# NVIDIA/k8s-operator-libs

Hardware: AMD Instinct MI355X
Metric: 8-node rolling-upgrade wall-clock (lower is better)
Workload: dtype fp32; 1 GPU; model=amdgpu-driver-rolling-upgrade, nodes_per_cluster=8, maxParallelUpgrades=2, maxUnavailable=50%, drain=True, podDeletion=True, gpu_pods_per_node=2, gpu_validation=True, converging_reconcile=True, mode=inplace, global_batch=8, parallelism=dp1 (one independent simulated 8-node cluster per rank)

## Files before the change

k8s_operator_libs_amd/core/restclient.py:

```python

from __future__ import annotations

import collections
import http.client as _http_client
import json
import os
from typing import Any, Dict, Optional

import httpx

from ..native import load_wire as _load_wire
from . import meta
from .client import Client
from .errors import (
    AlreadyExistsError,
    ApiError,
    BadRequestError,
    ConflictError,
    NotFoundError,
)

SA_DIR = "/var/run/secrets/kubernetes.io/serviceaccount"

_KIND_INFO = {
    ("v1", "Node"): ("nodes", False),
    ("v1", "Pod"): ("pods", True),
    ("v1", "Event"): ("events", True),
    ("v1", "Namespace"): ("namespaces", False),
    ("apps/v1", "DaemonSet"): ("daemonsets", True),
    ("apps/v1", "ControllerRevision"): ("controllerrevisions", True),
    ("apiextensions.k8s.io/v1", "CustomResourceDefinition"): (
        "customresourcedefinitions", False),
    ("maintenance.amd.com/v1alpha1", "NodeMaintenance"): ("nodemaintenances", True),
    ("coordination.k8s.io/v1", "Lease"): ("leases", True),
}


def _lower_plural(kind: str) -> str:
    k = kind.lower()
    if k.endswith(("ss", "x", "z", "ch", "sh")):
        return k + "es"
    if k.endswith("s"):
        return k
    if k.endswith("y") and len(k) > 1 and k[-2] not in "aeiou":
        return k[:-1] + "ies"
    return k + "s"


class RestClient(Client):
    def __init__(
        self,
        base_url: str,
        token: Optional[str] = None,
        verify: Any = True,
        timeout: float = 30.0,
        extra_kinds: Optional[Dict[tuple, tuple]] = None,
        retries: int = 3,
    ) -> None:
        self.base_url = base_url.rstrip("/")
        headers = {"Content-Type": "application/json"}
        if token:
            headers["Authorization"] = f"Bearer {token}"
        self._headers = dict(headers)
        self._timeout = timeout
        self._http = httpx.Client(
            base_url=self.base_url, headers=headers, verify=verify, timeout=timeout
        )
        self._fast_netloc = None
        self._wire = None
        if self.base_url.startswith("http://"):
            import urllib.parse

            parsed = urllib.parse.urlsplit(self.base_url)
            self._fast_netloc = (parsed.hostname, parsed.port or 80)
            self._fast_local = __import__("threading").local()
            self._wire = _load_wire()
            self._wire_heads: Dict[tuple, bytes] = {}
        self._kinds = dict(_KIND_INFO)
        if extra_kinds:
            self._kinds.update(extra_kinds)
        self._retries = retries


    def _wire_head(self, headers=None) -> bytes:
        key = tuple(sorted(headers.items())) if headers else ()
        head = self._wire_heads.get(key)
        if head is None:
            host, port = self._fast_netloc
            if ":" in host:
                host = f"[{host}]"
            hdrs = {"Host": host if port == 80 else f"{host}:{port}",
                    "Accept-Encoding": "identity"}
            hdrs.update(self._headers)
            if headers:
                hdrs.update(headers)
            head = "".join(f"{k}: {v}\r\n" for k, v in hdrs.items()).encode(
                "latin-1")
            self._wire_heads[key] = head
        return head

    def _wire_connect(self):
        import socket

        sock = socket.create_connection(self._fast_netloc,
                                        timeout=self._timeout)
        sock.setsockopt(socket.IPPROTO_TCP, socket.TCP_NODELAY, 1)
        return sock

    def _wire_request(self, method: str, path: str, params=None, content=None,
                      headers=None):
        import urllib.parse

        if params:
            path = f"{path}?{urllib.parse.urlencode(params)}"
        head = self._wire_head(headers)
        sock = getattr(self._fast_local, "sock", None)
        for attempt in (0, 1):
            try:
                if sock is None:
                    sock = self._wire_connect()
                    self._fast_local.sock = sock
                status, data, reusable = self._wire.exchange(
                    sock.fileno(), method, path, head, content, self._timeout)
            except ValueError as exc:
                self._wire_drop(sock)
                raise _http_client.HTTPException(str(exc)) from exc
            except (ConnectionError, OSError):
                self._wire_drop(sock)
                sock = None
                if attempt:
                    raise
            except BaseException:
                self._wire_drop(sock)
                raise
            else:
                if not reusable:
                    self._wire_drop(sock)
                return _FastResponse(status, data)
        raise AssertionError("unreachable")

    def _wire_drop(self, sock) -> None:
        if sock is not None:
            try:
                sock.close()
            except Exception:
                pass
        self._fast_local.sock = None

    def _fast_request(self, method: str, path: str, params=None, content=None,
                      headers=None):
        if self._wire is not None:
            return self._wire_request(method, path, params=params,
                                      content=content, headers=headers)
        import http.client
        import urllib.parse

        if params:
            path = f"{path}?{urllib.parse.urlencode(params)}"
        conn = getattr(self._fast_local, "conn", None)
        hdrs = dict(self._headers)
        if headers:
            hdrs.update(headers)
        body = content if content is not None else None
        for attempt in (0, 1):
            if conn is None:
                conn = http.client.HTTPConnection(
                    *self._fast_netloc, timeout=self._timeout
                )
                self._fast_local.conn = conn
            try:
                conn.request(method, path, body=body, headers=hdrs)
                resp = conn.getresponse()
                data = resp.read()
                return _FastResponse(resp.status, data)
            except (http.client.HTTPException, ConnectionError, OSError):
                try:
                    conn.close()
                except Exception:
                    pass
                conn = None
                self._fast_local.conn = None
                if attempt:
                    raise
        raise AssertionError("unreachable")

    def _request(self, method: str, path: str, **kw) -> httpx.Response:
        import time as _time

        attempt = 0
        while True:
            try:
                if self._fast_netloc is not None:
                    resp = self._fast_request(method, path, **kw)
                else:
                    resp = self._http.request(method, path, **kw)
            except (httpx.ConnectError, httpx.ReadError, httpx.RemoteProtocolError,
                    httpx.ConnectTimeout, httpx.ReadTimeout,
                    _http_client.HTTPException,
                    ConnectionError, OSError) as exc:
                if attempt >= self._retries:
                    err = ApiError(f"connection to apiserver failed: {exc}")
                    err.code = 503
                    raise err from exc
            else:
                if resp.status_code not in (429, 500, 502, 503, 504) or \
                        attempt >= self._retries:
                    return resp
            attempt += 1
            _time.sleep(min(0.05 * (2 ** attempt), 1.0))

    @classmethod
    def from_environment(cls) -> "RestClient":
        token_path = os.path.join(SA_DIR, "token")
        if os.path.exists(token_path):
            with open(token_path) as fh:
                token = fh.read().strip()
            host = os.environ.get("KUBERNETES_SERVICE_HOST", "kubernetes.default.svc")
            port = os.environ.get("KUBERNETES_SERVICE_PORT", "443")
            ca = os.path.join(SA_DIR, "ca.crt")
            return cls(f"https://{host}:{port}", token=token,
                       verify=ca if os.path.exists(ca) else True)
# ... 136 lines not shown
        return resp.json()

    def update(self, obj):
        api_version, kind = meta.api_version(obj), meta.kind(obj)
        path = self._object_path(api_version, kind, meta.name(obj), meta.namespace(obj))
        resp = self._request("PUT", path, content=json.dumps(obj))
        self._raise_for(resp)
        return resp.json()

    def patch(self, api_version, kind, name, patch, namespace=""):
        path = self._object_path(api_version, kind, name, namespace)
        resp = self._request(
            "PATCH", path, content=json.dumps(patch),
            headers={"Content-Type": "application/merge-patch+json"},
        )
        self._raise_for(resp)
        return resp.json()

    def delete(self, api_version, kind, name, namespace="", grace_period_seconds=None):
        kw = {}
        if grace_period_seconds is not None:
            kw["content"] = json.dumps({
                "apiVersion": "v1", "kind": "DeleteOptions",
                "gracePeriodSeconds": int(grace_period_seconds),
            })
        resp = self._request(
            "DELETE", self._object_path(api_version, kind, name, namespace), **kw
        )
        self._raise_for(resp)

    def patch_status(self, api_version, kind, name, status, namespace=""):
        path = self._object_path(api_version, kind, name, namespace) + "/status"
        resp = self._request(
            "PATCH", path, content=json.dumps({"status": status}),
            headers={"Content-Type": "application/merge-patch+json"},
        )
        self._raise_for(resp)
        return resp.json()

    def evict_pod(self, name, namespace):
        path = self._object_path("v1", "Pod", name, namespace) + "/eviction"
        body = {
            "apiVersion": "policy/v1",
            "kind": "Eviction",
            "metadata": {"name": name, "namespace": namespace},
        }
        resp = self._request("POST", path, content=json.dumps(body))
        self._raise_for(resp)

    def watch(self, api_version: str, kind: str, namespace=None,
              resource_version=None, label_selector="", field_selector="",
              send_initial_events=False):
        return _HttpWatch(self, api_version, kind, namespace=namespace,
                          resource_version=resource_version,
                          label_selector=label_selector,
                          field_selector=field_selector,
                          send_initial_events=send_initial_events)


    def discover_resource(self, api_version: str, plural: str) -> bool:
        prefix = f"/api/{api_version}" if "/" not in api_version else f"/apis/{api_version}"
        resp = self._request("GET", prefix)
        if resp.status_code != 200:
            return False
        for res in resp.json().get("resources", []):
            if res.get("name") == plural:
                return True
        return False

    def register_kind(self, api_version: str, kind: str, plural: str, namespaced: bool) -> None:
        self._kinds[(api_version, kind)] = (plural, namespaced)

    def close(self) -> None:
        self._http.close()
        if self._fast_netloc is not None:
            conn = getattr(self._fast_local, "conn", None)
            if conn is not None:
                try:
                    conn.close()
                except Exception:
                    pass
                self._fast_local.conn = None
            self._wire_drop(getattr(self._fast_local, "sock", None))


class _FastResponse:

    __slots__ = ("status_code", "_data")

    def __init__(self, status_code: int, data: bytes) -> None:
        self.status_code = status_code
        self._data = data

    def json(self):
        return json.loads(self._data)

    @property
    def text(self) -> str:
        return self._data.decode(errors="replace")


class _HttpWatch:

    USE_LINE_PUMP = True

    def __init__(self, client: RestClient, api_version: str, kind: str,
                 namespace=None, resource_version=None,
                 label_selector="", field_selector="",
                 send_initial_events=False) -> None:
        import queue
        import threading

        self._queue: "queue.Queue" = queue.Queue()
        self._stop = threading.Event()
        self._connected = threading.Event()
        path = client._collection_path(api_version, kind, namespace or "")
        params = {"watch": "true", "allowWatchBookmarks": "true"}
        if resource_version is not None:
            params["resourceVersion"] = str(resource_version)
        if label_selector:
            params["labelSelector"] = label_selector
        if field_selector:
            params["fieldSelector"] = field_selector
        if send_initial_events:
            params["sendInitialEvents"] = "true"
            params["resourceVersionMatch"] = "NotOlderThan"
        self._error: Optional[BaseException] = None

        def reader():
            try:
                with client._http.stream(
                    "GET", path, params=params, timeout=None,
                ) as resp:
                    self._resp = resp
                    if resp.status_code == 410:
                        from .errors import GoneError

                        self._error = GoneError("watch resume point expired")
                        return
                    if resp.status_code >= 400:
                        err = ApiError(f"watch rejected: HTTP {resp.status_code}")
                        err.code = resp.status_code
                        self._error = err
                        return
                    self._connected.set()
                    for line in resp.iter_lines():
                        if self._stop.is_set():
                            break
                        line = line.strip()
                        if not line:
                            continue
                        try:
                            event = json.loads(line)
                        except ValueError:
                            continue
                        self._queue.put((event.get("type"), event.get("object")))
            except Exception as exc:
                if not self._stop.is_set():
                    import logging as _logging

                    _logging.getLogger(__name__).warning(
                        "watch stream ended: %s", exc
                    )
            finally:
                self._connected.set()

# ... 237 lines not shown
```

k8s_operator_libs_amd/native/build.py:

```python

from __future__ import annotations

import os
import subprocess
import sysconfig

PKG_DIR = os.path.dirname(os.path.abspath(__file__))
SOURCE = os.path.join(PKG_DIR, "gpu_validator.hip")
OUTPUT = os.path.join(PKG_DIR, "_gpu_validator.so")
JSONOPS_SOURCE = os.path.join(PKG_DIR, "jsonops.cpp")
JSONOPS_OUTPUT = os.path.join(PKG_DIR, "_jsonops.so")
WIRE_SOURCES = (
    os.path.join(PKG_DIR, "wire.cpp"),
    os.path.join(PKG_DIR, "wire_core.hpp"),
    os.path.join(PKG_DIR, "wire_stream.hpp"),
)
WIRE_OUTPUT = os.path.join(PKG_DIR, "_wire.so")

HIPCC = os.environ.get("HIPCC", "/opt/rocm/bin/hipcc")
CXX = os.environ.get("CXX", "g++")


def validator_sources() -> list:
    wire = {os.path.basename(p) for p in WIRE_SOURCES}
    return [SOURCE] + sorted(
        os.path.join(PKG_DIR, name) for name in os.listdir(PKG_DIR)
        if name.endswith(".hpp") and name not in wire)


def is_built() -> bool:
    return os.path.exists(OUTPUT) and all(
        os.path.getmtime(OUTPUT) >= os.path.getmtime(src)
        for src in validator_sources())


def build_jsonops(force: bool = False, verbose: bool = False) -> str:
    if (
        not force
        and os.path.exists(JSONOPS_OUTPUT)
        and os.path.getmtime(JSONOPS_OUTPUT) >= os.path.getmtime(JSONOPS_SOURCE)
    ):
        return JSONOPS_OUTPUT
    cmd = [
        CXX, "-O3", "-std=c++17", "-fPIC", "-shared",
        f"-I{sysconfig.get_paths()['include']}",
        JSONOPS_SOURCE, "-o", JSONOPS_OUTPUT,
    ]
    if verbose:
        print(" ".join(cmd))
    subprocess.run(cmd, check=True, capture_output=not verbose)
    return JSONOPS_OUTPUT


def build_wire(force: bool = False, verbose: bool = False) -> str:
    if (
        not force
        and os.path.exists(WIRE_OUTPUT)
        and all(os.path.getmtime(WIRE_OUTPUT) >= os.path.getmtime(src)
                for src in WIRE_SOURCES)
    ):
        return WIRE_OUTPUT
    cmd = [
        CXX, "-O3", "-std=c++17", "-fPIC", "-shared", "-pthread",
        f"-I{sysconfig.get_paths()['include']}",
        WIRE_SOURCES[0], "-o", WIRE_OUTPUT,
    ]
    if verbose:
        print(" ".join(cmd))
    subprocess.run(cmd, check=True, capture_output=not verbose)
    return WIRE_OUTPUT


def build(force: bool = False, verbose: bool = False) -> str:
    build_jsonops(force=force, verbose=verbose)
    build_wire(force=force, verbose=verbose)
    if is_built() and not force:
        return OUTPUT
    import pybind11

    cmd = [
        HIPCC,
        "--offload-arch=gfx950",
        "-O3",
        "-std=c++17",
        "-fPIC",
        "-shared",
        f"-I{sysconfig.get_paths()['include']}",
        f"-I{pybind11.get_include()}",
        SOURCE,
        "-o",
        OUTPUT,
    ]
    if verbose:
        print(" ".join(cmd))
    subprocess.run(cmd, check=True, capture_output=not verbose)
    return OUTPUT

# ... 5 lines not shown
```

k8s_operator_libs_amd/native/wire.cpp:

```cpp

#define PY_SSIZE_T_CLEAN
#include <Python.h>

#include <atomic>
#include <cerrno>
#include <chrono>
#include <memory>
#include <mutex>
#include <new>
#include <string>
#include <system_error>
#include <thread>
#include <vector>

#include <fcntl.h>
#include <poll.h>
#include <sys/socket.h>
#include <sys/types.h>
#include <unistd.h>

#include "wire_core.hpp"
#include "wire_stream.hpp"

namespace {

constexpr size_t kRecvBuf = 64 * 1024;

using Clock = std::chrono::steady_clock;

struct Deadline {
  bool infinite;
  Clock::time_point at;

  explicit Deadline(double timeout_s) : infinite(timeout_s < 0) {
    if (!infinite)
      at = Clock::now() + std::chrono::duration_cast<Clock::duration>(
                              std::chrono::duration<double>(timeout_s));
  }

  int remaining_ms() const {
    if (infinite) return -1;
    auto left = std::chrono::duration_cast<std::chrono::microseconds>(
                    at - Clock::now()).count();
    if (left <= 0) return 0;
    long long ms = (left + 999) / 1000;
    return ms > 0x7fffffff ? 0x7fffffff : int(ms);
  }
};

bool parse_timeout(PyObject* obj, double* out) {
  if (obj == nullptr || obj == Py_None) {
    *out = -1.0;
    return true;
  }
  double v = PyFloat_AsDouble(obj);
  if (v == -1.0 && PyErr_Occurred()) return false;
  *out = v < 0 ? 0.0 : v;
  return true;
}

enum IoResult { kIoOk = 0, kIoTimeout = 1, kIoError = 2, kIoSignal = 3 };

IoResult wait_fd(int fd, short events, const Deadline& dl) {
  for (;;) {
    int ms = dl.remaining_ms();
    struct pollfd p = {fd, events, 0};
    int rc, err;
    Py_BEGIN_ALLOW_THREADS
    rc = poll(&p, 1, ms);
    err = errno;
    Py_END_ALLOW_THREADS
    if (rc > 0) return kIoOk;
    if (rc == 0) {
      if (ms != 0 && dl.remaining_ms() != 0) continue;
      return kIoTimeout;
    }
    if (err == EINTR) {
      if (PyErr_CheckSignals() < 0) return kIoSignal;
      continue;
    }
    errno = err;
    PyErr_SetFromErrno(PyExc_OSError);
    return kIoError;
  }
}

IoResult recv_some(int fd, char* buf, size_t cap, const Deadline& dl,
                   size_t* got) {
  for (;;) {
    int ms = dl.remaining_ms();
    struct pollfd p = {fd, POLLIN, 0};
    int rc, err;
    ssize_t n = -1;
    Py_BEGIN_ALLOW_THREADS
    rc = poll(&p, 1, ms);
    err = errno;
    if (rc > 0) {
      n = recv(fd, buf, cap, MSG_DONTWAIT);
      err = errno;
    }
    Py_END_ALLOW_THREADS
    if (rc == 0) {
      if (ms != 0 && dl.remaining_ms() != 0) continue;
      return kIoTimeout;
    }
    if (n >= 0) {
      *got = size_t(n);
      return kIoOk;
    }
    if (rc > 0 && (err == EAGAIN || err == EWOULDBLOCK)) continue;
    if (err == EINTR) {
      if (PyErr_CheckSignals() < 0) return kIoSignal;
      continue;
    }
    errno = err;
    PyErr_SetFromErrno(PyExc_OSError);
    return kIoError;
  }
}

IoResult send_all(int fd, const char* buf, size_t len, const Deadline& dl) {
  size_t off = 0;
  while (off < len) {
    ssize_t n;
    int err;
    Py_BEGIN_ALLOW_THREADS
    n = send(fd, buf + off, len - off, MSG_NOSIGNAL | MSG_DONTWAIT);
    err = errno;
    Py_END_ALLOW_THREADS
    if (n >= 0) {
      off += size_t(n);
      continue;
    }
    if (err == EAGAIN || err == EWOULDBLOCK) {
      IoResult w = wait_fd(fd, POLLOUT, dl);
      if (w != kIoOk) return w;
      continue;
    }
    if (err == EINTR) {
      if (PyErr_CheckSignals() < 0) return kIoSignal;
      continue;
    }
    errno = err;
    PyErr_SetFromErrno(PyExc_OSError);
    return kIoError;
  }
  return kIoOk;
}

PyObject* raise_wire_error(int st) {
  PyErr_SetString(PyExc_ValueError, wire::status_message(st));
  return nullptr;
}

PyObject* raise_timeout() {
  PyErr_SetString(PyExc_TimeoutError, "timed out");
  return nullptr;
}

bool status_has_no_body(int status) {
  return status == 204 || status == 304;
}

bool as_buffer(PyObject* obj, const char** p, Py_ssize_t* n, bool* present) {
  *present = true;
  if (obj == Py_None) {
    *p = "";
    *n = 0;
    *present = false;
    return true;
  }
  if (PyBytes_Check(obj)) {
    *p = PyBytes_AS_STRING(obj);
    *n = PyBytes_GET_SIZE(obj);
    return true;
  }
  if (PyUnicode_Check(obj)) {
    *p = PyUnicode_AsUTF8AndSize(obj, n);
    return *p != nullptr;
  }
  PyErr_SetString(PyExc_TypeError, "body must be bytes, str or None");
  return false;
}


PyObject* py_exchange(PyObject* , PyObject* args) {
  int fd;
  const char *method, *path, *head;
  Py_ssize_t method_len, path_len, head_len;
  PyObject *body_obj, *timeout_obj = Py_None;
  if (!PyArg_ParseTuple(args, "is#s#y#O|O", &fd, &method, &method_len, &path,
                        &path_len, &head, &head_len, &body_obj, &timeout_obj))
    return nullptr;
  const char* body;
  Py_ssize_t body_len;
  bool has_body;
  if (!as_buffer(body_obj, &body, &body_len, &has_body)) return nullptr;
  double timeout_s;
  if (!parse_timeout(timeout_obj, &timeout_s)) return nullptr;
  Deadline dl(timeout_s);

  std::string method_s(method, size_t(method_len));
  bool is_head = method_s == "HEAD";
  bool wants_length = has_body || method_s == "POST" || method_s == "PUT" ||
                      method_s == "PATCH";

  std::string req;
  req.reserve(size_t(method_len + path_len + head_len + body_len) + 64);
  req.append(method_s).append(" ").append(path, size_t(path_len));
  req.append(" HTTP/1.1\r\n").append(head, size_t(head_len));
  if (wants_length)
    req.append("Content-Length: ").append(std::to_string(body_len)).append("\r\n");
  req.append("\r\n").append(body, size_t(body_len));

  IoResult io = send_all(fd, req.data(), req.size(), dl);
  if (io == kIoTimeout) return raise_timeout();
  if (io != kIoOk) return nullptr;

  wire::HeadParser head_parser(wire::HeadParser::kResponse);
  wire::ChunkedDecoder chunked;
  std::string out;
  enum { kHead, kLength, kChunked, kUntilClose, kComplete } phase = kHead;
  size_t remaining = 0;
  bool reusable = true;
  bool got_any = false;
  char buf[kRecvBuf];

  while (phase != kComplete) {
    size_t got = 0;
    io = recv_some(fd, buf, sizeof buf, dl, &got);
    if (io == kIoTimeout) return raise_timeout();
    if (io != kIoOk) return nullptr;
    if (got == 0) {
      if (phase == kUntilClose) {
        phase = kComplete;
        break;
      }
      PyErr_SetString(got_any ? PyExc_ConnectionError
                              : PyExc_ConnectionResetError,
                      got_any ? "peer closed the connection mid-response"
                              : "peer closed the connection without a response");
      return nullptr;
    }
    got_any = true;
    const char* p = buf;
    size_t n = got;
    while (n > 0 && phase != kComplete) {
      size_t used = 0;
      if (phase == kHead) {
        int st = head_parser.feed(p, n, &used);
        if (st < 0) return raise_wire_error(st);
        if (st == wire::kDone) {
          int code = head_parser.status;
          if (code >= 100 && code < 200 && code != 101) {
            head_parser.reset();
          } else {
            if (!head_parser.keep_alive()) reusable = false;
            if (is_head || status_has_no_body(code)) {
              phase = kComplete;
            } else if (head_parser.chunked) {
              phase = kChunked;
            } else if (head_parser.has_content_length) {
              remaining = head_parser.content_length;
              if (remaining == 0) {
                phase = kComplete;
              } else {
                phase = kLength;
                out.reserve(remaining < (size_t(1) << 26) ? remaining
                                                          : (size_t(1) << 26));
              }
            } else {
              phase = kUntilClose;
              reusable = false;
            }
          }
        }
      } else if (phase == kLength) {
        used = n < remaining ? n : remaining;
        out.append(p, used);
        remaining -= used;
        if (remaining == 0) phase = kComplete;
      } else if (phase == kChunked) {
        int st = chunked.feed(p, n, &used, &out);
        if (st < 0) return raise_wire_error(st);
        if (st == wire::kDone) phase = kComplete;
      } else {
        used = n;
        out.append(p, used);
      }
      p += used;
      n -= used;
    }
    if (n > 0) reusable = false;
  }

  PyObject* body_bytes =
      PyBytes_FromStringAndSize(out.data(), Py_ssize_t(out.size()));
  if (!body_bytes) return nullptr;
  PyObject* res = Py_BuildValue("(iNO)", head_parser.status, body_bytes,
                                reusable ? Py_True : Py_False);
  return res;
}


PyObject* py_parse_request_head(PyObject* , PyObject* arg) {
  Py_buffer view;
  if (PyObject_GetBuffer(arg, &view, PyBUF_SIMPLE) < 0) return nullptr;
  wire::HeadParser hp(wire::HeadParser::kRequest);
  size_t used = 0;
  int st = hp.feed(static_cast<const char*>(view.buf), size_t(view.len), &used);
  PyBuffer_Release(&view);
  if (st < 0) return raise_wire_error(st);
  if (st == wire::kNeedMore) Py_RETURN_NONE;
  PyObject* length;
  if (hp.has_content_length) {
    length = PyLong_FromSize_t(hp.content_length);
    if (!length) return nullptr;
  } else {
    length = Py_None;
    Py_INCREF(length);
  }
  return Py_BuildValue("(s#s#iNOOn)", hp.method.data(),
                       Py_ssize_t(hp.method.size()), hp.target.data(),
                       Py_ssize_t(hp.target.size()), hp.version_minor, length,
                       hp.chunked ? Py_True : Py_False,
                       hp.keep_alive() ? Py_True : Py_False,
                       Py_ssize_t(used));
}


struct LineReaderObject {
  PyObject_HEAD
  int fd;
  bool busy;
  wire::LineFramer* framer;
  std::string* buf;
};

void linereader_dealloc(LineReaderObject* self) {
  delete self->framer;
  delete self->buf;
  Py_TYPE(self)->tp_free(reinterpret_cast<PyObject*>(self));
}

int linereader_init(LineReaderObject* self, PyObject* args, PyObject* ) {
  int fd;
  if (!PyArg_ParseTuple(args, "i", &fd)) return -1;
  if (self->framer != nullptr) {
    PyErr_SetString(PyExc_RuntimeError, "LineReader is already initialised");
    return -1;
  }
  self->fd = fd;
  self->busy = false;
  try {
    self->framer = new wire::LineFramer();
    self->buf = new std::string(kRecvBuf, '\0');
  } catch (const std::bad_alloc&) {
    PyErr_NoMemory();
    return -1;
  }
  return 0;
}

IoResult linereader_fill(LineReaderObject* self, const Deadline& dl) {
  size_t got = 0;
  self->busy = true;
  IoResult io = recv_some(self->fd, &(*self->buf)[0], self->buf->size(), dl,
                          &got);
  self->busy = false;
  if (io != kIoOk) return io;
  if (got == 0) {
    self->framer->peer_closed();
    return kIoOk;
  }
  try {
    int st = self->framer->consume(self->buf->data(), got);
    if (st < 0) {
      raise_wire_error(st);
      return kIoError;
    }
  } catch (const std::bad_alloc&) {
    PyErr_NoMemory();
    return kIoError;
// ... 568 lines not shown
        std::make_shared<Stream>(fd, size_t(max_backlog)));
  } catch (const std::bad_alloc&) {
    PyErr_NoMemory();
    return -1;
  }
  self->closed = false;
  return 0;
}

PyObject* streamwriter_write(StreamWriterObject* self, PyObject* arg) {
  if (self->stream == nullptr) {
    PyErr_SetString(PyExc_RuntimeError, "StreamWriter is not initialised");
    return nullptr;
  }
  Py_buffer view;
  if (PyObject_GetBuffer(arg, &view, PyBUF_SIMPLE) < 0) return nullptr;
  bool ok = false;
  if (!self->closed) {
    const std::shared_ptr<Stream>& s = *self->stream;
    Stream* raw = s.get();
    try {
      auto st = raw->buf.write(
          static_cast<const char*>(view.buf), size_t(view.len),
          [raw](const char* p, size_t n) { return raw->send_some(p, n); });
      if (st == wire::StreamBuffer::kQueued && !Flusher::instance().attach(s)) {
        raw->buf.kill();
        st = wire::StreamBuffer::kDead;
      }
      if (st == wire::StreamBuffer::kDead) raw->on_dead();
      ok = st != wire::StreamBuffer::kDead;
    } catch (const std::bad_alloc&) {
      raw->buf.kill();
      raw->on_dead();
    }
  }
  PyBuffer_Release(&view);
  return PyBool_FromLong(ok);
}

PyObject* streamwriter_close(StreamWriterObject* self, PyObject*) {
  if (self->stream != nullptr && !self->closed) {
    self->closed = true;
    Flusher::instance().detach(*self->stream);
  }
  Py_RETURN_NONE;
}

PyObject* streamwriter_get_dead(StreamWriterObject* self, void*) {
  if (self->stream == nullptr) Py_RETURN_TRUE;
  return PyBool_FromLong(self->closed || (*self->stream)->buf.dead());
}

PyObject* streamwriter_get_pending(StreamWriterObject* self, void*) {
  if (self->stream == nullptr) return PyLong_FromLong(0);
  return PyLong_FromSize_t((*self->stream)->buf.pending());
}

PyMethodDef streamwriter_methods[] = {
    {"write", reinterpret_cast<PyCFunction>(streamwriter_write), METH_O,
     "write(data) -> bool.  Thread-safe, never blocks, never raises for a "
     "broken stream.  With nothing queued the bytes are sent on the calling "
     "thread; what the socket does not take waits in the backlog, which one "
     "native thread per process drains on POLLOUT.  Each call's bytes reach "
     "the peer contiguously.  False once the writer is dead or closed."},
    {"close", reinterpret_cast<PyCFunction>(streamwriter_close), METH_NOARGS,
     "close().  Detach from the flusher thread; on return nothing native "
     "uses the fd any more.  Unsent backlog is dropped."},
    {nullptr, nullptr, 0, nullptr},
};

PyGetSetDef streamwriter_getset[] = {
    {"dead", reinterpret_cast<getter>(streamwriter_get_dead), nullptr,
     "True after a send error, a backlog past max_backlog (the socket is "
     "then shut down, not closed) or close()", nullptr},
    {"pending", reinterpret_cast<getter>(streamwriter_get_pending), nullptr,
     "bytes waiting in the backlog", nullptr},
    {nullptr, nullptr, nullptr, nullptr, nullptr},
};

PyTypeObject StreamWriterType = {
    PyVarObject_HEAD_INIT(nullptr, 0)
    "_wire.StreamWriter",
    sizeof(StreamWriterObject),
};


PyObject* py_exchange_guarded(PyObject* self, PyObject* args) {
  try {
    return py_exchange(self, args);
  } catch (const std::bad_alloc&) {
    return PyErr_NoMemory();
  }
}

PyObject* py_parse_request_head_guarded(PyObject* self, PyObject* arg) {
  try {
    return py_parse_request_head(self, arg);
  } catch (const std::bad_alloc&) {
    return PyErr_NoMemory();
  }
}

PyMethodDef wire_methods[] = {
    {"exchange", py_exchange_guarded, METH_VARARGS,
     "exchange(fd, method, path, header_bytes, body, timeout=None) -> "
     "(status, body_bytes, reusable).  One HTTP/1.1 request/response on a "
     "connected socket: the request goes out in a single send; the response "
     "is read with Content-Length, chunked or read-to-EOF framing.  "
     "reusable is False when the connection must not carry another request."},
    {"parse_request_head", py_parse_request_head_guarded, METH_O,
     "parse_request_head(data) -> None | (method, target, minor_version, "
     "content_length | None, chunked, keep_alive, head_size).  None while "
     "the head is incomplete; ValueError when it is malformed."},
    {nullptr, nullptr, 0, nullptr},
};

struct PyModuleDef wire_module = {
    PyModuleDef_HEAD_INIT, "_wire",
    "Native HTTP/1.1 framing for the REST client and the watch reader", -1,
    wire_methods,
};

}

PyMODINIT_FUNC PyInit__wire(void) {
  LineReaderType.tp_flags = Py_TPFLAGS_DEFAULT;
  LineReaderType.tp_doc =
      "LineReader(fd): newline-delimited reader over a streaming HTTP "
      "response on a socket the caller owns (never closed here).";
  LineReaderType.tp_new = PyType_GenericNew;
  LineReaderType.tp_init = reinterpret_cast<initproc>(linereader_init);
  LineReaderType.tp_dealloc = reinterpret_cast<destructor>(linereader_dealloc);
  LineReaderType.tp_methods = linereader_methods;
  LineReaderType.tp_getset = linereader_getset;
  if (PyType_Ready(&LineReaderType) < 0) return nullptr;
  StreamWriterType.tp_flags = Py_TPFLAGS_DEFAULT;
  StreamWriterType.tp_doc =
      "StreamWriter(fd, max_backlog=64 MiB): non-blocking, thread-safe line "
      "writer over a socket the caller owns (never closed here).  The "
      "default cap holds the replay that opens a watch, which is written in "
      "one go, and equals the 64 MiB cap on a single line; a reader further "
      "behind than that is cut off and re-watches.";
  StreamWriterType.tp_new = PyType_GenericNew;
  StreamWriterType.tp_init = reinterpret_cast<initproc>(streamwriter_init);
  StreamWriterType.tp_dealloc =
      reinterpret_cast<destructor>(streamwriter_dealloc);
  StreamWriterType.tp_methods = streamwriter_methods;
  StreamWriterType.tp_getset = streamwriter_getset;
  if (PyType_Ready(&StreamWriterType) < 0) return nullptr;
  LinePumpType.tp_flags = Py_TPFLAGS_DEFAULT;
  LinePumpType.tp_doc =
      "LinePump(fd | LineReader): one native thread reads the response head "
      "and then lines from a socket the caller owns, without ever taking "
      "the GIL; consumers wait() for the line count to move and drain().  "
      "Given a LineReader, the thread reads through it and the reader is "
      "the pump's from then on.  To end it: shut the socket down, stop(), "
      "and only then close the socket.";
  LinePumpType.tp_new = PyType_GenericNew;
  LinePumpType.tp_init = reinterpret_cast<initproc>(linepump_init);
  LinePumpType.tp_dealloc = reinterpret_cast<destructor>(linepump_dealloc);
  LinePumpType.tp_methods = linepump_methods;
  LinePumpType.tp_getset = linepump_getset;
  if (PyType_Ready(&LinePumpType) < 0) return nullptr;
  PyObject* m = PyModule_Create(&wire_module);
  if (!m) return nullptr;
  Py_INCREF(&LinePumpType);
  if (PyModule_AddObject(m, "LinePump",
                         reinterpret_cast<PyObject*>(&LinePumpType)) < 0) {
    Py_DECREF(&LinePumpType);
    Py_DECREF(m);
    return nullptr;
  }
  Py_INCREF(&StreamWriterType);
  if (PyModule_AddObject(m, "StreamWriter",
                         reinterpret_cast<PyObject*>(&StreamWriterType)) < 0) {
    Py_DECREF(&StreamWriterType);
    Py_DECREF(m);
    return nullptr;
  }
  Py_INCREF(&LineReaderType);
  if (PyModule_AddObject(m, "LineReader",
                         reinterpret_cast<PyObject*>(&LineReaderType)) < 0) {
    Py_DECREF(&LineReaderType);
    Py_DECREF(m);
    return nullptr;
  }
  return m;
}
```

k8s_operator_libs_amd/native/wire_core.hpp:

```cpp

#pragma once

#include <cstddef>
#include <cstdint>
#include <cstring>
#include <string>

namespace wire {

enum Status : int {
  kNeedMore = 0,
  kDone = 1,
  kErrHeadTooLarge = -1,
  kErrBadHead = -2,
  kErrBadLength = -3,
  kErrBadChunk = -4,
  kErrLineTooLong = -5,
};

inline const char* status_message(int st) {
  switch (st) {
    case kNeedMore: return "need more input";
    case kDone: return "done";
    case kErrHeadTooLarge: return "HTTP head larger than 64 KiB";
// ... 239 lines not shown
            state_ = kSizeLF;
          } else if (c == ';' || detail::is_ows(c)) {
            state_ = kExt;
          } else {
            return fail(consumed, i);
          }
          if (++meta_len_ > kMaxHead) return fail(consumed, i);
          break;
        }
        case kExt:
          if (c == '\r') state_ = kSizeLF;
          else if (c == '\n') return fail(consumed, i);
          if (++meta_len_ > kMaxHead) return fail(consumed, i);
          break;
        case kSizeLF:
          if (c != '\n') return fail(consumed, i);
          meta_len_ = 0;
          if (remaining_ == 0) {
            state_ = kTrailer;
            trailer_line_len_ = 0;
          } else {
            state_ = kData;
          }
          break;
        case kDataCR:
          if (c != '\r') return fail(consumed, i);
          state_ = kDataLF;
          break;
        case kDataLF:
          if (c != '\n') return fail(consumed, i);
          state_ = kSizeFirst;
          break;
        case kTrailer:
          if (c == '\r') state_ = kTrailerLF;
          else if (c == '\n') return fail(consumed, i);
          else ++trailer_line_len_;
          if (++meta_len_ > kMaxHead) return fail(consumed, i);
          break;
        case kTrailerLF:
          if (c != '\n') return fail(consumed, i);
          if (trailer_line_len_ == 0) {
            state_ = kEnd;
          } else {
            state_ = kTrailer;
            trailer_line_len_ = 0;
          }
          break;
        default:
          return fail(consumed, i);
      }
    }
    *consumed = i;
    return state_ == kEnd ? kDone : kNeedMore;
  }

  bool done() const { return state_ == kEnd; }

 private:
  enum State {
    kSizeFirst, kSize, kExt, kSizeLF, kData, kDataCR, kDataLF,
    kTrailer, kTrailerLF, kEnd, kFailed,
  };

  static int hex(char c) {
    if (c >= '0' && c <= '9') return c - '0';
    if (c >= 'a' && c <= 'f') return c - 'a' + 10;
    if (c >= 'A' && c <= 'F') return c - 'A' + 10;
    return -1;
  }

  int fail(size_t* consumed, size_t i) {
    state_ = kFailed;
    *consumed = i;
    return kErrBadChunk;
  }

  State state_;
  size_t remaining_;
  size_t meta_len_;
  size_t trailer_line_len_;
};


class LineSplitter {
 public:
  explicit LineSplitter(size_t max_line = kMaxLine)
      : max_line_(max_line), pos_(0), scan_(0) {}

  void feed(const char* data, size_t n) {
    if (pos_ > 0 && pos_ == buf_.size()) {
      buf_.clear();
      pos_ = scan_ = 0;
    }
    buf_.append(data, n);
  }

  int next(std::string* out) {
    for (;;) {
      const char* base = buf_.data();
      const char* lf = scan_ < buf_.size()
          ? static_cast<const char*>(
                std::memchr(base + scan_, '\n', buf_.size() - scan_))
          : nullptr;
      if (!lf) {
        scan_ = buf_.size();
        if (buf_.size() - pos_ > max_line_) return kErrLineTooLong;
        if (pos_ > 0) {
          buf_.erase(0, pos_);
          scan_ -= pos_;
          pos_ = 0;
        }
        return kNeedMore;
      }
      size_t end = size_t(lf - base);
      size_t start = pos_;
      pos_ = scan_ = end + 1;
      if (end - start > max_line_) return kErrLineTooLong;
      if (strip(base, start, end, out)) return kDone;
    }
  }

  int flush(std::string* out) {
    size_t start = pos_, end = buf_.size();
    pos_ = scan_ = end;
    if (end - start > max_line_) return kErrLineTooLong;
    return strip(buf_.data(), start, end, out) ? kDone : kNeedMore;
  }

  size_t pending() const { return buf_.size() - pos_; }

 private:
  static bool is_space(char c) {
    return c == ' ' || c == '\t' || c == '\r' || c == '\n' || c == '\f' ||
           c == '\v';
  }

  static bool strip(const char* base, size_t start, size_t end,
                    std::string* out) {
    while (start < end && is_space(base[start])) ++start;
    while (end > start && is_space(base[end - 1])) --end;
    if (start == end) return false;
    out->assign(base + start, end - start);
    return true;
  }

  size_t max_line_;
  std::string buf_;
  size_t pos_;
  size_t scan_;
};

}
```

Before: 25.12 ms.

## Share keep-alive connections across threads via a native connection pool

Adds a native C++ Pool that keeps idle keep-alive sockets to the API server and lends them to any thread. Before, each thread kept its own socket. Threads in the concurrent drain, pod and node workers can now reuse warm connections instead of dialing new TCP connections, and the idle count is sized from the worker concurrency limits. Response parsing moves into a reusable ResponseReader class. The change adds mutex contention, a poll per checkout to detect stale sockets, and retry logic for reset connections.

```diff
diff --git a/k8s_operator_libs_amd/core/restclient.py b/k8s_operator_libs_amd/core/restclient.py
--- a/k8s_operator_libs_amd/core/restclient.py
+++ b/k8s_operator_libs_amd/core/restclient.py
@@ -47,7 +47,19 @@
     return k + "s"
 
 
+def _pool_max_idle() -> int:
+    from ..upgrade.common_manager import CommonUpgradeManager
+    from ..upgrade.drain_manager import DrainManager
+    from ..upgrade.pod_manager import PodManager
+
+    return (1 + PodManager.MAX_CONCURRENT_NODE_WORKERS
+            + DrainManager.MAX_CONCURRENT_NODE_WORKERS
+            + CommonUpgradeManager.MAX_PARALLEL_NODE_OPS)
+
+
 class RestClient(Client):
+    USE_POOL = True
+
     def __init__(
         self,
         base_url: str,
@@ -68,6 +80,7 @@
         )
         self._fast_netloc = None
         self._wire = None
+        self._pool = None
         if self.base_url.startswith("http://"):
             import urllib.parse
 
@@ -76,6 +89,10 @@
             self._fast_local = __import__("threading").local()
             self._wire = _load_wire()
             self._wire_heads: Dict[tuple, bytes] = {}
+            if self._wire is not None and hasattr(self._wire, "Pool"):
+                self._pool = self._wire.Pool(
+                    *self._fast_netloc, max_idle=_pool_max_idle(),
+                    connect_timeout=timeout)
         self._kinds = dict(_KIND_INFO)
         if extra_kinds:
             self._kinds.update(extra_kinds)
@@ -114,6 +131,12 @@
         if params:
             path = f"{path}?{urllib.parse.urlencode(params)}"
         head = self._wire_head(headers)
+        pool = self._pool if self.USE_POOL else None
+        if pool is not None:
+            try:
+                return self._pool_request(pool, method, path, head, content)
+            except _PoolClosed:
+                pass
         sock = getattr(self._fast_local, "sock", None)
         for attempt in (0, 1):
             try:
@@ -137,6 +160,28 @@
                 if not reusable:
                     self._wire_drop(sock)
                 return _FastResponse(status, data)
+        raise AssertionError("unreachable")
+
+    def _pool_request(self, pool, method: str, path: str, head: bytes,
+                      content):
+        for fresh in (False, True):
+            try:
+                fd, reused = pool.checkout(fresh)
+            except RuntimeError as exc:
+                raise _PoolClosed() from exc
+            keep = False
+            try:
+                status, data, keep = self._wire.exchange(
+                    fd, method, path, head, content, self._timeout)
+            except ValueError as exc:
+                raise _http_client.HTTPException(str(exc)) from exc
+            except (ConnectionResetError, BrokenPipeError):
+                if not reused:
+                    raise
+            else:
+                return _FastResponse(status, data)
+            finally:
+                pool.checkin(fd, keep)
         raise AssertionError("unreachable")
 
     def _wire_drop(self, sock) -> None:
@@ -439,6 +484,13 @@
                     pass
                 self._fast_local.conn = None
             self._wire_drop(getattr(self._fast_local, "sock", None))
+            pool, self._pool = self._pool, None
+            if pool is not None:
+                pool.close()
+
+
+class _PoolClosed(Exception):
+    """The client was closed while a request was on its way to the pool."""
 
 
 class _FastResponse:
diff --git a/k8s_operator_libs_amd/native/build.py b/k8s_operator_libs_amd/native/build.py
--- a/k8s_operator_libs_amd/native/build.py
+++ b/k8s_operator_libs_amd/native/build.py
@@ -13,6 +13,7 @@
 WIRE_SOURCES = (
     os.path.join(PKG_DIR, "wire.cpp"),
     os.path.join(PKG_DIR, "wire_core.hpp"),
+    os.path.join(PKG_DIR, "wire_pool.hpp"),
     os.path.join(PKG_DIR, "wire_stream.hpp"),
 )
 WIRE_OUTPUT = os.path.join(PKG_DIR, "_wire.so")
diff --git a/k8s_operator_libs_amd/native/wire.cpp b/k8s_operator_libs_amd/native/wire.cpp
--- a/k8s_operator_libs_amd/native/wire.cpp
+++ b/k8s_operator_libs_amd/native/wire.cpp
@@ -20,6 +20,7 @@
 #include <unistd.h>
 
 #include "wire_core.hpp"
+#include "wire_pool.hpp"
 #include "wire_stream.hpp"
 
 namespace {
@@ -156,10 +157,6 @@
 PyObject* raise_timeout() {
   PyErr_SetString(PyExc_TimeoutError, "timed out");
   return nullptr;
-}
-
-bool status_has_no_body(int status) {
-  return status == 204 || status == 304;
 }
 
 bool as_buffer(PyObject* obj, const char** p, Py_ssize_t* n, bool* present) {
@@ -217,88 +214,33 @@
   if (io == kIoTimeout) return raise_timeout();
   if (io != kIoOk) return nullptr;
 
-  wire::HeadParser head_parser(wire::HeadParser::kResponse);
-  wire::ChunkedDecoder chunked;
-  std::string out;
-  enum { kHead, kLength, kChunked, kUntilClose, kComplete } phase = kHead;
-  size_t remaining = 0;
-  bool reusable = true;
-  bool got_any = false;
+  wire::ResponseReader reader(is_head);
   char buf[kRecvBuf];
 
-  while (phase != kComplete) {
+  while (!reader.done()) {
     size_t got = 0;
     io = recv_some(fd, buf, sizeof buf, dl, &got);
     if (io == kIoTimeout) return raise_timeout();
     if (io != kIoOk) return nullptr;
     if (got == 0) {
-      if (phase == kUntilClose) {
-        phase = kComplete;
-        break;
-      }
+      if (reader.peer_closed()) break;
+      bool got_any = reader.started();
       PyErr_SetString(got_any ? PyExc_ConnectionError
                               : PyExc_ConnectionResetError,
                       got_any ? "peer closed the connection mid-response"
                               : "peer closed the connection without a response");
       return nullptr;
     }
-    got_any = true;
-    const char* p = buf;
-    size_t n = got;
-    while (n > 0 && phase != kComplete) {
-      size_t used = 0;
-      if (phase == kHead) {
-        int st = head_parser.feed(p, n, &used);
-        if (st < 0) return raise_wire_error(st);
-        if (st == wire::kDone) {
-          int code = head_parser.status;
-          if (code >= 100 && code < 200 && code != 101) {
-            head_parser.reset();
-          } else {
-            if (!head_parser.keep_alive()) reusable = false;
-            if (is_head || status_has_no_body(code)) {
-              phase = kComplete;
-            } else if (head_parser.chunked) {
-              phase = kChunked;
-            } else if (head_parser.has_content_length) {
-              remaining = head_parser.content_length;
-              if (remaining == 0) {
-                phase = kComplete;
-              } else {
-                phase = kLength;
-                out.reserve(remaining < (size_t(1) << 26) ? remaining
-                                                          : (size_t(1) << 26));
-              }
-            } else {
-              phase = kUntilClose;
-              reusable = false;
-            }
-          }
-        }
-      } else if (phase == kLength) {
-        used = n < remaining ? n : remaining;
-        out.append(p, used);
-        remaining -= used;
-        if (remaining == 0) phase = kComplete;
-      } else if (phase == kChunked) {
-        int st = chunked.feed(p, n, &used, &out);
-        if (st < 0) return raise_wire_error(st);
-        if (st == wire::kDone) phase = kComplete;
-      } else {
-        used = n;
-        out.append(p, used);
-      }
-      p += used;
-      n -= used;
-    }
-    if (n > 0) reusable = false;
-  }
-
+    int st = reader.feed(buf, got);
+    if (st < 0) return raise_wire_error(st);
+  }
+
+  const std::string& out = reader.body();
   PyObject* body_bytes =
       PyBytes_FromStringAndSize(out.data(), Py_ssize_t(out.size()));
   if (!body_bytes) return nullptr;
-  PyObject* res = Py_BuildValue("(iNO)", head_parser.status, body_bytes,
-                                reusable ? Py_True : Py_False);
+  PyObject* res = Py_BuildValue("(iNO)", reader.status(), body_bytes,
+                                reader.reusable() ? Py_True : Py_False);
   return res;
 }
 
@@ -1033,6 +975,189 @@
     PyVarObject_HEAD_INIT(nullptr, 0)
     "_wire.StreamWriter",
     sizeof(StreamWriterObject),
+};
+
+
+struct PoolObject {
+  PyObject_HEAD
+  wire::Pool* pool;
+};
+
+void pool_dealloc(PoolObject* self) {
+  delete self->pool;
+  Py_TYPE(self)->tp_free(reinterpret_cast<PyObject*>(self));
+}
+
+int pool_init(PoolObject* self, PyObject* args, PyObject* kw) {
+  static const char* names[] = {"host", "port", "max_idle", "connect_timeout",
+                                nullptr};
+  const char* host;
+  int port;
+  Py_ssize_t max_idle = 8;
+  PyObject* timeout_obj = Py_None;
+  if (!PyArg_ParseTupleAndKeywords(args, kw, "si|nO",
+                                   const_cast<char**>(names), &host, &port,
+                                   &max_idle, &timeout_obj))
+    return -1;
+  if (self->pool != nullptr) {
+    PyErr_SetString(PyExc_RuntimeError, "Pool is already initialised");
+    return -1;
+  }
+  if (port < 0 || port > 65535 || max_idle < 0) {
+    PyErr_SetString(PyExc_ValueError,
+                    "port must be 0..65535 and max_idle >= 0");
+    return -1;
+  }
+  double timeout_s;
+  if (!parse_timeout(timeout_obj, &timeout_s)) return -1;
+  try {
+    self->pool = new wire::Pool(host, port, size_t(max_idle), timeout_s);
+  } catch (const std::bad_alloc&) {
+    PyErr_NoMemory();
+    return -1;
+  }
+  return 0;
+}
+
+bool pool_enter(PoolObject* self) {
+  if (self->pool == nullptr) {
+    PyErr_SetString(PyExc_RuntimeError, "Pool is not initialised");
+    return false;
+  }
+  return true;
+}
+
+bool pool_on_eintr(void*) {
+  PyGILState_STATE gil = PyGILState_Ensure();
+  bool go_on = PyErr_CheckSignals() == 0;
+  PyGILState_Release(gil);
+  return go_on;
+}
+
+PyObject* pool_checkout_impl(PoolObject* self, PyObject* args) {
+  int fresh = 0;
+  if (!PyArg_ParseTuple(args, "|p", &fresh)) return nullptr;
+  if (!pool_enter(self)) return nullptr;
+  wire::Pool::Lease lease;
+  if (!fresh) lease = self->pool->take_idle();
+  if (lease.fd < 0 && lease.error == wire::Pool::kOk) {
+    Py_BEGIN_ALLOW_THREADS
+    lease = self->pool->dial(pool_on_eintr, nullptr);
+    Py_END_ALLOW_THREADS
+  }
+  switch (lease.error) {
+    case wire::Pool::kOk:
+      return Py_BuildValue("(iO)", lease.fd,
+                           lease.reused ? Py_True : Py_False);
+    case wire::Pool::kClosed:
+      PyErr_SetString(PyExc_RuntimeError, "Pool is closed");
+      return nullptr;
+    case wire::Pool::kResolve: {
+      PyObject* gaierror = nullptr;
+      PyObject* mod = PyImport_ImportModule("socket");
+      if (mod != nullptr) {
+        gaierror = PyObject_GetAttrString(mod, "gaierror");
+        Py_DECREF(mod);
+      }
+      if (gaierror == nullptr) return nullptr;
+      PyObject* val = Py_BuildValue("(is)", lease.code, gai_strerror(lease.code));
+      if (val != nullptr) {
+        PyErr_SetObject(gaierror, val);
+        Py_DECREF(val);
+      }
+      Py_DECREF(gaierror);
+      return nullptr;
+    }
+    case wire::Pool::kTimeout:
+      return raise_timeout();
+    case wire::Pool::kInterrupted:
+      return nullptr;
+    default:
+      errno = lease.code;
+      return PyErr_SetFromErrno(PyExc_OSError);
+  }
+}
+
+PyObject* pool_checkout(PoolObject* self, PyObject* args) {
+  try {
+    return pool_checkout_impl(self, args);
+  } catch (const std::bad_alloc&) {
+    return PyErr_NoMemory();
+  }
+}
+
+PyObject* pool_checkin(PoolObject* self, PyObject* args) {
+  int fd, reusable;
+  if (!PyArg_ParseTuple(args, "ip", &fd, &reusable)) return nullptr;
+  if (!pool_enter(self)) return nullptr;
+  try {
+    self->pool->checkin(fd, reusable != 0);
+  } catch (const std::bad_alloc&) {
+    close(fd);
+  }
+  Py_RETURN_NONE;
+}
+
+PyObject* pool_close(PoolObject* self, PyObject*) {
+  if (!pool_enter(self)) return nullptr;
+  self->pool->close();
+  Py_RETURN_NONE;
+}
+
+PyObject* pool_stats(PoolObject* self, PyObject*) {
+  if (!pool_enter(self)) return nullptr;
+  wire::PoolStats st = self->pool->stats();
+  return Py_BuildValue("{s:K,s:K,s:K,s:n}", "dials",
+                       static_cast<unsigned long long>(st.dials), "reuses",
+                       static_cast<unsigned long long>(st.reuses),
+                       "stale_discards",
+                       static_cast<unsigned long long>(st.stale_discards),
+                       "idle", Py_ssize_t(st.idle));
+}
+
+PyObject* pool_get_max_idle(PoolObject* self, void*) {
+  if (!pool_enter(self)) return nullptr;
+  return PyLong_FromSize_t(self->pool->max_idle());
+}
+
+PyObject* pool_get_closed(PoolObject* self, void*) {
+  if (!pool_enter(self)) return nullptr;
+  return PyBool_FromLong(self->pool->closed());
+}
+
+PyMethodDef pool_methods[] = {
+    {"checkout", reinterpret_cast<PyCFunction>(pool_checkout), METH_VARARGS,
+     "checkout(fresh=False) -> (fd, reused).  The most recently used idle "
+     "connection that is still quiet (reused=True), else (or with fresh) a "
+     "new one, dialled with the GIL released.  The fd stays the pool's: pass it to exchange() and "
+     "give it back with checkin(), exactly once, never close it.  OSError "
+     "(TimeoutError, socket.gaierror) when the dial fails; RuntimeError "
+     "once the pool is closed."},
+    {"checkin", reinterpret_cast<PyCFunction>(pool_checkin), METH_VARARGS,
+     "checkin(fd, reusable).  Give a checked-out fd back.  It is kept for "
+     "the next checkout() only when reusable is true (the response was "
+     "complete and exchange() said reusable), the pool is open and fewer "
+     "than max_idle are idle; otherwise the pool closes it."},
+    {"close", reinterpret_cast<PyCFunction>(pool_close), METH_NOARGS,
+     "close().  Close the idle connections; one checked out now is closed "
+     "when it comes back.  checkout() raises from here on."},
+    {"stats", reinterpret_cast<PyCFunction>(pool_stats), METH_NOARGS,
+     "stats() -> {'dials', 'reuses', 'stale_discards', 'idle'}."},
+    {nullptr, nullptr, 0, nullptr},
+};
+
+PyGetSetDef pool_getset[] = {
+    {"max_idle", reinterpret_cast<getter>(pool_get_max_idle), nullptr,
+     "most connections kept idle", nullptr},
+    {"closed", reinterpret_cast<getter>(pool_get_closed), nullptr,
+     "True after close()", nullptr},
+    {nullptr, nullptr, nullptr, nullptr, nullptr},
+};
+
+PyTypeObject PoolType = {
+    PyVarObject_HEAD_INIT(nullptr, 0)
+    "_wire.Pool",
+    sizeof(PoolObject),
 };
 
 
@@ -1113,8 +1238,28 @@
   LinePumpType.tp_methods = linepump_methods;
   LinePumpType.tp_getset = linepump_getset;
   if (PyType_Ready(&LinePumpType) < 0) return nullptr;
+  PoolType.tp_flags = Py_TPFLAGS_DEFAULT;
+  PoolType.tp_doc =
+      "Pool(host, port, max_idle=8, connect_timeout=None): keep-alive "
+      "connections to one plain-HTTP endpoint, shared by every thread.  The "
+      "pool opens its sockets itself and is the only one to close them; "
+      "checkout() lends an fd to one exchange() at a time.  A forked child "
+      "starts with an empty pool.";
+  PoolType.tp_new = PyType_GenericNew;
+  PoolType.tp_init = reinterpret_cast<initproc>(pool_init);
+  PoolType.tp_dealloc = reinterpret_cast<destructor>(pool_dealloc);
+  PoolType.tp_methods = pool_methods;
+  PoolType.tp_getset = pool_getset;
+  if (PyType_Ready(&PoolType) < 0) return nullptr;
   PyObject* m = PyModule_Create(&wire_module);
   if (!m) return nullptr;
+  Py_INCREF(&PoolType);
+  if (PyModule_AddObject(m, "Pool",
+                         reinterpret_cast<PyObject*>(&PoolType)) < 0) {
+    Py_DECREF(&PoolType);
+    Py_DECREF(m);
+    return nullptr;
+  }
   Py_INCREF(&LinePumpType);
   if (PyModule_AddObject(m, "LinePump",
                          reinterpret_cast<PyObject*>(&LinePumpType)) < 0) {
diff --git a/k8s_operator_libs_amd/native/wire_core.hpp b/k8s_operator_libs_amd/native/wire_core.hpp
--- a/k8s_operator_libs_amd/native/wire_core.hpp
+++ b/k8s_operator_libs_amd/native/wire_core.hpp
@@ -345,6 +345,94 @@
 };
 
 
+class ResponseReader {
+ public:
+  explicit ResponseReader(bool head_request)
+      : head_(HeadParser::kResponse), head_request_(head_request) {}
+
+  int feed(const char* p, size_t n) {
+    if (n > 0) started_ = true;
+    while (n > 0 && phase_ != kComplete) {
+      size_t used = 0;
+      if (phase_ == kHead) {
+        int st = head_.feed(p, n, &used);
+        if (st < 0) return st;
+        if (st == kDone) on_head();
+      } else if (phase_ == kLength) {
+        used = n < remaining_ ? n : remaining_;
+        body_.append(p, used);
+        remaining_ -= used;
+        if (remaining_ == 0) phase_ = kComplete;
+      } else if (phase_ == kChunked) {
+        int st = chunked_.feed(p, n, &used, &body_);
+        if (st < 0) return st;
+        if (st == kDone) phase_ = kComplete;
+      } else {
+        used = n;
+        body_.append(p, used);
+      }
+      p += used;
+      n -= used;
+    }
+    if (n > 0) reusable_ = false;
+    return phase_ == kComplete ? kDone : kNeedMore;
+  }
+
+  bool peer_closed() {
+    if (phase_ == kUntilClose) phase_ = kComplete;
+    return phase_ == kComplete;
+  }
+
+  bool done() const { return phase_ == kComplete; }
+  bool started() const { return started_; }
+  int status() const { return head_.status; }
+  bool reusable() const { return reusable_; }
+  std::string& body() { return body_; }
+
+ private:
+  static bool status_has_no_body(int status) {
+    return status == 204 || status == 304;
+  }
+
+  void on_head() {
+    int code = head_.status;
+    if (code >= 100 && code < 200 && code != 101) {
+      head_.reset();
+      return;
+    }
+    if (!head_.keep_alive()) reusable_ = false;
+    if (head_request_ || status_has_no_body(code)) {
+      phase_ = kComplete;
+    } else if (head_.chunked) {
+      phase_ = kChunked;
+    } else if (head_.has_content_length) {
+      remaining_ = head_.content_length;
+      if (remaining_ == 0) {
+        phase_ = kComplete;
+      } else {
+        phase_ = kLength;
+        body_.reserve(remaining_ < (size_t(1) << 26) ? remaining_
+                                                     : (size_t(1) << 26));
+      }
+    } else {
+      phase_ = kUntilClose;
+      reusable_ = false;
+    }
+  }
+
+  enum Phase { kHead, kLength, kChunked, kUntilClose, kComplete };
+
+  HeadParser head_;
+  ChunkedDecoder chunked_;
+  std::string body_;
+  Phase phase_ = kHead;
+  size_t remaining_ = 0;
+  bool head_request_;
+  bool reusable_ = true;
+  bool started_ = false;
+};
+
+
 class LineSplitter {
  public:
   explicit LineSplitter(size_t max_line = kMaxLine)
diff --git a/k8s_operator_libs_amd/native/wire_pool.hpp b/k8s_operator_libs_amd/native/wire_pool.hpp
--- /dev/null
+++ b/k8s_operator_libs_amd/native/wire_pool.hpp
@@ -0,0 +1,260 @@
+
+#pragma once
+
+#include <cerrno>
+#include <chrono>
+#include <cstdint>
+#include <cstdio>
+#include <mutex>
+#include <string>
+#include <vector>
+
+#include <netdb.h>
+#include <netinet/in.h>
+#include <netinet/tcp.h>
+#include <poll.h>
+#include <sys/socket.h>
+#include <sys/types.h>
+#include <unistd.h>
+
+namespace wire {
+
+struct PoolStats {
+  uint64_t dials = 0;
+  uint64_t reuses = 0;
+  uint64_t stale_discards = 0;
+  size_t idle = 0;
+};
+
+class Pool {
+ public:
+  enum Error {
+    kOk = 0,
+    kClosed,
+    kResolve,
+    kConnect,
+    kTimeout,
+    kInterrupted,
+  };
+
+  struct Lease {
+    int fd = -1;
+    bool reused = false;
+    Error error = kOk;
+    int code = 0;
+  };
+
+  using OnEintr = bool (*)(void*);
+
+  Pool(std::string host, int port, size_t max_idle, double connect_timeout_s)
+      : host_(std::move(host)), port_(port), max_idle_(max_idle),
+        connect_timeout_s_(connect_timeout_s < 0 || connect_timeout_s > 1e6
+                               ? 1e6 : connect_timeout_s),
+        pid_(getpid()) {}
+
+  ~Pool() { close(); }
+
+  Pool(const Pool&) = delete;
+  Pool& operator=(const Pool&) = delete;
+
+  Lease take_idle() {
+    Lease lease;
+    for (;;) {
+      int fd;
+      {
+        std::lock_guard<std::mutex> hold(mu_);
+        after_fork();
+        if (closed_) {
+          lease.error = kClosed;
+          return lease;
+        }
+        if (idle_.empty()) return lease;
+        fd = idle_.back();
+        idle_.pop_back();
+      }
+      struct pollfd p = {fd, POLLIN | POLLRDHUP | POLLHUP | POLLERR, 0};
+      int rc = poll(&p, 1, 0);
+      if (rc == 0) {
+        std::lock_guard<std::mutex> hold(mu_);
+        ++stats_.reuses;
+        lease.fd = fd;
+        lease.reused = true;
+        return lease;
+      }
+      ::close(fd);
+      std::lock_guard<std::mutex> hold(mu_);
+      ++stats_.stale_discards;
+    }
+  }
+
+  Lease dial(OnEintr on_eintr = nullptr, void* arg = nullptr) {
+    Lease lease;
+    {
+      std::lock_guard<std::mutex> hold(mu_);
+      after_fork();
+      if (closed_) {
+        lease.error = kClosed;
+        return lease;
+      }
+    }
+    char service[16];
+    std::snprintf(service, sizeof service, "%d", port_);
+    struct addrinfo hints = {};
+    hints.ai_socktype = SOCK_STREAM;
+    hints.ai_flags = AI_NUMERICHOST | AI_NUMERICSERV;
+    struct addrinfo* found = nullptr;
+    int rc = getaddrinfo(host_.c_str(), service, &hints, &found);
+    if (rc == EAI_NONAME) {
+      hints.ai_flags = AI_NUMERICSERV;
+      rc = getaddrinfo(host_.c_str(), service, &hints, &found);
+    }
+    if (rc != 0) {
+      lease.error = kResolve;
+      lease.code = rc;
+      return lease;
+    }
+    auto deadline = std::chrono::steady_clock::now() +
+                    std::chrono::duration_cast<std::chrono::microseconds>(
+                        std::chrono::duration<double>(connect_timeout_s_));
+    lease.error = kConnect;
+    lease.code = EADDRNOTAVAIL;
+    for (struct addrinfo* ai = found; ai != nullptr; ai = ai->ai_next) {
+      int fd = socket(ai->ai_family, ai->ai_socktype | SOCK_NONBLOCK | SOCK_CLOEXEC,
+                      ai->ai_protocol);
+      if (fd < 0) {
+        lease.code = errno;
+        continue;
+      }
+      Error err = connect_fd(fd, ai, deadline, on_eintr, arg, &lease.code);
+      if (err == kOk) {
+        int one = 1;
+        setsockopt(fd, IPPROTO_TCP, TCP_NODELAY, &one, sizeof one);
+        lease.fd = fd;
+        lease.error = kOk;
+        lease.code = 0;
+        break;
+      }
+      ::close(fd);
+      lease.error = err;
+      if (err != kConnect) break;
+    }
+    freeaddrinfo(found);
+    if (lease.fd >= 0) {
+      std::lock_guard<std::mutex> hold(mu_);
+      ++stats_.dials;
+      if (closed_) {
+        ::close(lease.fd);
+        lease.fd = -1;
+        lease.error = kClosed;
+      }
+    }
+    return lease;
+  }
+
+  Lease checkout(OnEintr on_eintr = nullptr, void* arg = nullptr) {
+    Lease lease = take_idle();
+    if (lease.fd >= 0 || lease.error != kOk) return lease;
+    return dial(on_eintr, arg);
+  }
+
+  void checkin(int fd, bool reusable) {
+    if (fd < 0) return;
+    {
+      std::lock_guard<std::mutex> hold(mu_);
+      if (reusable && !closed_ && pid_ == getpid() &&
+          idle_.size() < max_idle_) {
+        idle_.push_back(fd);
+        return;
+      }
+    }
+    ::close(fd);
+  }
+
+  void close() {
+    std::vector<int> doomed;
+    {
+      std::lock_guard<std::mutex> hold(mu_);
+      after_fork();
+      closed_ = true;
+      doomed.swap(idle_);
+    }
+    for (int fd : doomed) ::close(fd);
+  }
+
+  bool closed() {
+    std::lock_guard<std::mutex> hold(mu_);
+    return closed_;
+  }
+
+  PoolStats stats() {
+    std::lock_guard<std::mutex> hold(mu_);
+    after_fork();
+    PoolStats out = stats_;
+    out.idle = idle_.size();
+    return out;
+  }
+
+  const std::string& host() const { return host_; }
+  int port() const { return port_; }
+  size_t max_idle() const { return max_idle_; }
+
+ private:
+  void after_fork() {
+    pid_t now = getpid();
+    if (now == pid_) return;
+    pid_ = now;
+    for (int fd : idle_) ::close(fd);
+    idle_.clear();
+    stats_ = PoolStats();
+  }
+
+  static Error connect_fd(int fd, const struct addrinfo* ai,
+                          std::chrono::steady_clock::time_point deadline,
+                          OnEintr on_eintr, void* arg, int* code) {
+    for (;;) {
+      if (connect(fd, ai->ai_addr, ai->ai_addrlen) == 0) return kOk;
+      if (errno == EINTR) {
+        if (on_eintr && !on_eintr(arg)) return kInterrupted;
+        break;
+      }
+      if (errno == EINPROGRESS) break;
+      *code = errno;
+      return kConnect;
+    }
+    for (;;) {
+      auto left = std::chrono::duration_cast<std::chrono::milliseconds>(
+                      deadline - std::chrono::steady_clock::now()).count();
+      if (left <= 0) return kTimeout;
+      struct pollfd p = {fd, POLLOUT, 0};
+      int rc = poll(&p, 1, left > 0x7fffffff ? 0x7fffffff : int(left) + 1);
+      if (rc < 0) {
+        if (errno != EINTR) {
+          *code = errno;
+          return kConnect;
+        }
+        if (on_eintr && !on_eintr(arg)) return kInterrupted;
+        continue;
+      }
+      if (rc == 0) continue;
+      int soerr = 0;
+      socklen_t len = sizeof soerr;
+      if (getsockopt(fd, SOL_SOCKET, SO_ERROR, &soerr, &len) != 0) soerr = errno;
+      if (soerr == 0) return kOk;
+      *code = soerr;
+      return kConnect;
+    }
+  }
+
+  const std::string host_;
+  const int port_;
+  const size_t max_idle_;
+  const double connect_timeout_s_;
+
+  std::mutex mu_;
+  pid_t pid_;
+  bool closed_ = false;
+  std::vector<int> idle_;
+  PoolStats stats_;
+};
+
+}
```

Result: faster. 22.32 ms, median of 6 (-11.1%).
